# fudan-zvg/PARTNER

Measured on AMD Instinct MI355X. Metric: frames/sec polar voxelize+PFN+BEV+head, 30k-pt sweep (whole job), higher is better.
Workload: dtype f32

## Files before the change

### include/partner_hip.h

```cpp
#ifndef PARTNER_HIP_H
#define PARTNER_HIP_H

#include <stddef.h>
#include <stdint.h>

#ifdef __cplusplus
extern "C" {
#endif

#define PN_OK 0
#define PN_ERR_INVALID (-1)
#define PN_ERR_LAUNCH (-2)
#define PN_ERR_WORKSPACE (-3)

#define PN_ACT_NONE 0
#define PN_ACT_RELU 1
#define PN_ACT_TANH 2
#define PN_ACT_GELU 3

typedef void *pn_stream_t;

int pn_version(void);
int pn_last_error(char *buf, size_t buf_len);
int pn_device_count(void);
// ... 564 lines not shown
size_t pn_pillar_conv_packed_weight_floats(int cout, int cin);
int pn_pack_pillar_conv_weight_f32(const float *w_oihw, int cout, int cin, float *packed, pn_stream_t stream);
size_t pn_pillar_conv_workspace_bytes(int v_capacity, int batch, int oh, int ow, int cout);
int pn_pillar_conv3x3_f32(const float *canvas, int batch, int h, int w, int cin, int in_pixel_stride, int in_channel_offset,
                          const uint32_t *unq_keys, const int32_t *num_voxels, int v_capacity, int stride,
                          const float *packed_w, int cout, const float *scale, const float *shift, int act, float *out,
                          int out_pixel_stride, int out_channel_offset, void *workspace, size_t workspace_bytes,
                          pn_stream_t stream);
int pn_pillar_conv_planes_supported(int batch, int oh, int ow, int cout);
int pn_pillar_conv3x3_planes_f32(const float *canvas, int batch, int h, int w, int cin, int in_pixel_stride, int in_channel_offset,
                                 const uint32_t *unq_keys, const int32_t *num_voxels, int v_capacity, int stride,
                                 const float *packed_w, int cout, const float *scale, const float *shift, int act, float *planes,
                                 void *workspace, size_t workspace_bytes, pn_stream_t stream);
int pn_pillar_conv_rows_supported(int batch, int h, int w, int cin, int cout, int stride);
size_t pn_pillar_conv_rows_packed_weight_floats(int cout, int cin);
int pn_pack_pillar_conv_rows_weight_f32(const float *w_oihw, int cout, int cin, float *packed, pn_stream_t stream);
int pn_pillar_conv3x3_rows_f32(const float *canvas, int batch, int h, int w, int cin, int in_pixel_stride, int in_channel_offset,
                               const uint32_t *unq_keys, const int32_t *row_start, int v_capacity, const float *packed_rows_w, int cout,
                               const float *scale, const float *shift, int act, float *planes, float *out, int out_pixel_stride,
                               int out_channel_offset, pn_stream_t stream);
int pn_conv2d_nhwc_planes_supported(const pn_conv_desc *d);
int pn_conv2d_nhwc_planes_f32(const pn_conv_desc *d, const float *in, const float *packed_w, const float *scale, const float *shift,
                              float *planes, pn_stream_t stream);
size_t pn_pillar_pairs_bytes(int v_capacity, int batch, int oh, int ow);
int pn_pillar_pairs_build(const uint32_t *unq_keys, const int32_t *num_voxels, int v_capacity, int batch, int h, int w,
                          int stride, void *pair_tables, size_t table_bytes, pn_stream_t stream);
int pn_pillar_conv3x3_tables_f32(const float *canvas, int batch, int oh, int ow, int cin, int in_pixel_stride,
                                 int in_channel_offset, const void *pair_tables, int v_capacity, const float *packed_w,
                                 int cout, const float *scale, const float *shift, int act, float *out,
                                 int out_pixel_stride, int out_channel_offset, void *workspace, size_t workspace_bytes,
                                 pn_stream_t stream);
int pn_pillar_conv3x3_dgrad_f32(const float *dout, int batch, int oh, int ow, int cout, int dout_pixel_stride,
                                int dout_channel_offset, const void *pair_tables, const int32_t *num_voxels,
                                int v_capacity, const float *packed_wt, int cin, float *dfeat, void *workspace,
                                size_t workspace_bytes, pn_stream_t stream);
size_t pn_pillar_conv_wgrad_workspace_bytes(int v_capacity, int cin, int cout);
int pn_pillar_conv3x3_wgrad_f32(const float *canvas, int in_pixel_stride, int in_channel_offset, int cin, const float *dout,
                                int dout_pixel_stride, int dout_channel_offset, int cout, const void *pair_tables,
                                int v_capacity, int batch, int oh, int ow, float *dw_oihw, int accumulate, void *workspace,
                                size_t workspace_bytes, pn_stream_t stream);
size_t pn_conv_stat_partial_floats(const pn_conv_desc *desc, int tile);
int pn_conv2d_multi_f32(const pn_conv_job *jobs, int njobs, int tile, pn_stream_t stream);
int pn_conv2d_small_n_multi_f32(const pn_conv_job *jobs, int njobs, pn_stream_t stream);

int pn_conv3x3_tap_sum_f32(const float *g, int ldg, int batch, int h, int w, int cout, const float *scale,
                           const float *shift, int act, float *out, int out_pixel_stride,
// ... 53 lines not shown
```

### partner_amd/autodiff.py

```python
from __future__ import annotations

import os

import ctypes as C
from typing import Callable, List, Optional, Sequence

import torch

from . import hip, ops
from .routes import R


class Node:
    __slots__ = ("v", "g", "bw", "owned", "name", "needs_grad")

    def __init__(self, v: torch.Tensor, bw: Optional[Callable] = None, name: Optional[str] = None, needs_grad=True):
        self.v, self.bw, self.name, self.needs_grad = v, bw, name, needs_grad
        self.g: Optional[torch.Tensor] = None
        self.owned = False


class Tape:
    def __init__(self):
        self.nodes: List[Node] = []
# ... 304 lines not shown

    def bw(dy):
        dx = torch.empty_like(dy)
        hip.call("pn_l2_normalize_bwd_f32", y.data_ptr(), dy.data_ptr(), inv.data_ptr(), rows, c, float(eps), dx.data_ptr(), hip.stream())
        accumulate(x, dx, own=True)

    return t.new(y, bw)


def _pad4(dy: torch.Tensor) -> torch.Tensor:
    c = dy.shape[-1]
    if c % 4 == 0:
        return dy
    out = torch.zeros(dy.shape[:-1] + ((c + 3) // 4 * 4,), dtype=torch.float32, device=dy.device)
    out[..., :c].copy_(dy)
    return out




def conv2d(t: Tape, x: Node, w: Node, b: Optional[Node], stride=1, pad=0, relu=False) -> Node:
    wv = w.v
    cout, cin, k, _ = wv.shape
    layer = ops.ConvLayer(wv, stride=stride, pad=pad, shift=None if b is None else b.v, act=ops.ACT_RELU if relu else ops.ACT_NONE, wino4=R.train_wino4_max_pixels > 0)
    layer.wino4_max_pixels = R.train_wino4_max_pixels
    ct = x.v.shape[3]
    if ct != cin:
        layer.pad_input_channels(ct)
    y = layer(x.v)

    def bw(dy):
        if relu:
            dy = ops.relu_bwd(y, dy)
        dy4 = _pad4(dy)
        def weight_grads():
            dw = ops.conv_wgrad(x.v, dy4, k, k, stride, pad, cin=cin, cout=cout)
            accumulate(w, dw, own=True)
            if b is not None:
                accumulate(b, ops.channel_sum(dy4, c=cout), own=True)

        side_run(weight_grads, dy4, x.v)
        if x.needs_grad:
            dx = ops.ConvDgrad(wv, stride, pad)(dy4)
            if ct != cin:
                full = torch.zeros_like(x.v)
                full[..., :cin].copy_(dx)
                dx = full
# ... 131 lines not shown
```

### partner_amd/hip.py

```python
from __future__ import annotations

import ctypes as C
import os
from typing import Optional

import torch

_LIB_PATH = os.path.join(os.path.dirname(os.path.abspath(__file__)), "lib", "libpartner_hip.so")
_lib: Optional[C.CDLL] = None

ACT_NONE, ACT_RELU, ACT_TANH, ACT_GELU = 0, 1, 2, 3


class PartnerHipError(RuntimeError):
    pass


class ConvDesc(C.Structure):

    _fields_ = [(n, C.c_int32) for n in (
        "batch", "in_h", "in_w", "cin", "cout", "groups", "kh", "kw", "stride", "pad_h", "pad_w",
        "in_pixel_stride", "in_channel_offset", "out_pixel_stride", "out_channel_offset", "act", "deconv2x2",
        "range_strata", "pad_h_end", "pad_w_end", "accumulate", "frames_in_flight", "transpose_hw")]

# ... 156 lines not shown
                                      _F, _P, _F, _F, _F, _P, _P, _P, _P, _P, _P, _P, _P, _SZ, _P]),
    "pn_rotate_boxes_f32": (_I, [_P, _P, _I, _I, _I, C.c_double, _P]),
    "pn_split_polar_sectors_workspace_bytes": (_SZ, [_I, _I, _I]),
    "pn_split_polar_sectors_f32": (_I, [_P, _I, _I, _P, _I, _I, _P, _P, _P, _P, _P, _P, _P, _P, _SZ, _P]),
    "pn_assemble_rows_f32": (_I, [C.POINTER(RowPiece), _I, _I, _I, _I, _P, _I, _I, _P]),
    "pn_sparse_neighbors_transpose": (_I, [_P, _P, _I, _I, _I, _P, _P]),
    "pn_sparse_conv_wgrad_workspace_bytes": (_SZ, [_I, _I, _I, _I]),
    "pn_sparse_conv_wgrad_f32": (_I, [_P, _I, _I, _I, _P, _I, _P, _P, _I, _I, _P, _I, _P, _SZ, _P]),
    "pn_sparse_from_dense_nhwc": (_I, [_P, _P, _I, _P, _P, _I, _P, _P]),
    "pn_add_relu_f32": (_I, [_P, _P, _P, _SZ, _P]),
    "pn_pad_roll_f32": (_I, [_P, _I, _I, _I, _I, _I, _I, _I, _P, _P]),
    "pn_crop_roll_f32": (_I, [_P, _I, _I, _I, _I, _I, _I, _I, _P, _P]),
    "pn_scale_channels_f32": (_I, [_P, _P, _SZ, _I, _P, _P]),
    "pn_recip_clamp_f32": (_I, [_P, _F, _I, _P, _P]),
    "pn_recip_clamp_bwd_f32": (_I, [_P, _P, _F, _I, _P, _P]),
    "pn_global_augment_f32": (_I, [_P, _I, _I, _P, _I, _I, _I, _I, _I, _F, _F, _F, _F, _P, _P]),
    "pn_handle_create": (_I, [_I, _P]),
    "pn_handle_destroy": (_I, [_P]),
    "pn_handle_info": (_I, [_P, _P, _P, _P, _P, _P, _SZ]),
    "pn_handle_pci_bus_id": (_I, [_P, _P, _SZ]),
    "pn_conv3x3_tap_sum_f32": (_I, [_P, _I, _I, _I, _I, _I, _P, _P, _I, _P, _I, _I, _P]),
    "pn_conv2d_nhwc_planes_supported": (_I, [_P]),
    "pn_conv2d_nhwc_planes_f32": (_I, [_P, _P, _P, _P, _P, _P, _P]),
    "pn_comm_unique_id_bytes": (_SZ, []),
    "pn_comm_unique_id": (_I, [_P]),
    "pn_comm_create": (_I, [_P, _I, _I, _P]),
    "pn_comm_destroy": (_I, [_P]),
    "pn_allreduce_f32": (_I, [_P, _P, _P, _SZ, _I, _P]),
    "pn_broadcast_f32": (_I, [_P, _P, _SZ, _I, _P]),
    "pn_linear_packed_weight_floats": (_SZ, [_I, _I]),
    "pn_pack_linear_weight_f32": (_I, [_P, _I, _I, _P, _P]),
    "pn_linear_set_tile": (_I, [_I]),
    "pn_linear_f32": (_I, [_P, _I, _I, _I, _P, _I, _P, _I, _P, _I, _P, _I, _P]),
    "pn_linear_ksplit_f32": (_I, [_P, _I, _I, _I, _P, _I, _P, _I, _P, _I, _P, _I, _P]),
    "pn_linear_ln_f32": (_I, [_P, _I, _I, _I, _P, _I, _P, _I, _P, _I, _P, _I, _P, _P, _F, _P, _P]),
    "pn_conv_wino_packed_weight_floats": (_SZ, [_I, _I]),
    "pn_pack_conv_weight_wino_f32": (_I, [_P, _I, _I, _P, _P]),
    "pn_pack_conv_dgrad_weight_wino_f32": (_I, [_P, _I, _I, _P, _P]),
    "pn_pack_conv_dgrad_weight_wino4_f32": (_I, [_P, _I, _I, _P, _P]),
    "pn_conv2d_wino_nhwc_f32": (_I, [_P, _P, _P, _P, _P, _P, _P]),
    "pn_conv_wino4_packed_weight_floats": (_SZ, [_I, _I]),
    "pn_pack_conv_weight_wino4_f32": (_I, [_P, _I, _I, _P, _P]),
    "pn_conv_wino4_tiles": (_I, [_P]),
    "pn_conv2d_wino4_nhwc_f32": (_I, [_P, _P, _P, _P, _P, _P, _P]),
    "pn_wino4_planes_floats": (_SZ, [_I, _I, _I, _I]),
    "pn_wino4_planes_from_nhwc_f32": (_I, [_P, _I, _I, _I, _I, _I, _I, _I, _P, _P]),
# ... 140 lines not shown
```

### partner_amd/ops_conv.py

```python
from __future__ import annotations

import ctypes as C
from dataclasses import dataclass
from typing import Optional, Sequence, Tuple

import torch

from . import hip
from .hip import ACT_NONE, ACT_RELU, ACT_TANH, ConvDesc
from .ops_common import *
from .ops_common import _f32, _workspace
from .routes import R, S
from .ops_index import VoxelIndex



class frames_in_flight:

    def __init__(self, n: int):
        self.n, self.prev = max(1, int(n)), 1

    def __enter__(self):
        self.prev, S.frames_in_flight = S.frames_in_flight, self.n
        return self
# ... 57 lines not shown


def disable_conv_profiling() -> None:
    S.profiler = None


def _tap_pack(buf: torch.Tensor, tap_n: int, cout: int, cin: int):
    def pack(w, st):
        w9 = torch.zeros((tap_n, cin), dtype=torch.float32, device=w.device)
        w9[:9 * cout] = w.reshape(cout, -1, 9)[:, :cin].permute(2, 0, 1).reshape(9 * cout, -1)
        hip.call("pn_pack_linear_weight_f32", w9.data_ptr(), tap_n, cin, buf.data_ptr(), st)
    return pack


def _transposed_pack(layout: str, buf: torch.Tensor, cout: int, cin: int, keep: dict):
    def pack(w, st):
        keep[layout] = wt = w.detach().float().transpose(2, 3).contiguous()
        hip.call(f"pn_pack_conv_weight_{layout}_f32", wt.data_ptr(), cout, cin, buf.data_ptr(), st)
    return pack




class ConvLayer:

    def __init__(self, weight: torch.Tensor, stride=1, pad=0, groups=1, scale=None, shift=None, act=ACT_NONE,
                 deconv2x2=False, range_strata=0, dtype="f32", wino4=True):
        hip.require_device(weight)
        lib = hip.load()
        w = weight.detach().contiguous().float()
        dev = w.device
        st = hip.stream()
        self.deconv2x2, self.range_strata, self.groups = bool(deconv2x2), int(range_strata), int(groups)
        self.stride, self.act = int(stride), int(act)
        self.pad = (pad, pad) if isinstance(pad, int) else tuple(pad)
        assert dtype in ("f32", "bf16")
        self.dtype = dtype
        self.packed_rows = self.wino44_packed = None
        self.wino4_max_pixels = None
        self._chain_t, self._chain_t_src = {}, {}
        self._packs = PackedLayouts(w)
        if dtype == "bf16":
            if deconv2x2:
                cin, cout = w.shape[0], w.shape[1]
                assert tuple(w.shape[2:]) == (2, 2)
                self.cin, self.cout, self.kh, self.kw = cin, cout, 1, 1
                wc = w.permute(2, 3, 1, 0).reshape(4 * cout, cin, 1, 1).contiguous()
                self.packed = torch.empty(lib.pn_conv_packed_weight_bf16_elems(4 * cout, cin, 1, 1, 1), dtype=torch.bfloat16, device=dev)
                hip.call("pn_pack_conv_weight_bf16", wc.data_ptr(), 4 * cout, cin, 1, 1, 1, self.packed.data_ptr(), st)
                self._pack_bf16_rows(lib, wc, 4 * cout, cin, 1, 1, st)
            else:
                pack_groups = self.range_strata if self.range_strata > 1 else self.groups
                cout_t, cin_g, kh, kw = w.shape
                self.cin, self.cout, self.kh, self.kw = cin_g, cout_t // pack_groups, kh, kw
                self.packed = None
                self._bf16_general = (w, cout_t, cin_g, kh, kw, pack_groups)
                if pack_groups == 1:
                    self._pack_bf16_rows(lib, w, cout_t, cin_g, kh, kw, st)
                if self.packed_rows is None:
                    self._ensure_bf16_general()
        elif deconv2x2:
# ... 12 lines not shown
        self.shift = None if shift is None else shift.detach().contiguous().float()
        self.out_channels = self.cout * (self.groups if not deconv2x2 else 1)
        self._pack_cin = self.cin
        self.wino_packed = None
        if (dtype == "f32" and not deconv2x2 and self.range_strata <= 1 and self.groups == 1 and (self.kh, self.kw) == (3, 3)
                and self.stride == 1 and self.pad == (1, 1) and self.cin % 4 == 0 and R.conv_wino):
            self.wino_packed = _f32(lib.pn_conv_wino_packed_weight_floats(self.cout, self.cin), dev)
            self._packs.add("wino", pack_call("pn_pack_conv_weight_wino_f32", self.wino_packed, self.cout, self.cin), now=True)
        self.wino4_packed = None
        if self.wino_packed is not None and R.conv_wino4 and wino4 and self.cout % 32 == 0 and self.act in (ACT_NONE, ACT_RELU):
            self.wino4_packed = _f32(lib.pn_conv_wino4_packed_weight_floats(self.cout, self.cin), dev)
            self._packs.add("wino4", pack_call("pn_pack_conv_weight_wino4_f32", self.wino4_packed, self.cout, self.cin), now=True)
        self.wino24_packed = None
        if self.wino4_packed is not None and R.conv_chain2d and self.cin % 32 == 0:
            self.wino24_packed = _f32(lib.pn_conv_wino24_packed_weight_floats(self.cout, self.cin), dev)
            self._packs.add("wino24", pack_call("pn_pack_conv_weight_wino24_f32", self.wino24_packed, self.cout, self.cin), now=True)

        self.tap_packed = None
        if (dtype == "f32" and not deconv2x2 and self.range_strata <= 1 and self.groups == 1 and (self.kh, self.kw) == (3, 3) and self.stride == 1
                and self.pad == (1, 1) and self.cout <= 3 and self.cin >= 128 and self.cin % 4 == 0 and R.conv_tapsum and R.linear):
            self.tap_n = (9 * self.cout + 3) // 4 * 4
            self.tap_packed = _f32(lib.pn_linear_packed_weight_floats(self.tap_n, self.cin), dev)
            self._packs.add("tap", _tap_pack(self.tap_packed, self.tap_n, self.cout, self.cin), now=True)
        if self.wino24_packed is None:
            self._packs.weight = None

    def _ensure_bf16_general(self) -> None:
        if self.packed is None:
            w, cout_t, cin_g, kh, kw, pack_groups = self._bf16_general
            self.packed = torch.empty(hip.load().pn_conv_packed_weight_bf16_elems(self.cout, cin_g, kh, kw, pack_groups), dtype=torch.bfloat16,
                                      device=w.device)
            hip.call("pn_pack_conv_weight_bf16", w.data_ptr(), cout_t, cin_g, kh, kw, pack_groups, self.packed.data_ptr(), hip.stream())

    def _pack_bf16_rows(self, lib, w: torch.Tensor, rows: int, cin: int, kh: int, kw: int, st) -> None:
        if cin % 64 == 0 and self.cout % 16 == 0 and self.act in (ACT_NONE, ACT_RELU):
            self.packed_rows = torch.empty(lib.pn_conv_bf16_rows_packed_elems(rows, cin, kh, kw), dtype=torch.bfloat16, device=w.device)
            hip.call("pn_pack_conv_weight_bf16_rows", w.data_ptr(), rows, cin, kh, kw, self.packed_rows.data_ptr(), st)

    def planes_desc(self, b: int, h: int, w: int, ct: int, in_channel_offset: int = 0):
        if self.dtype != "f32" or self.deconv2x2 or self.range_strata > 1 or self.groups != 1 or not R.conv_planes:
            return None
        d = ConvDesc(b, h, w, self.cin, self.cout, 1, self.kh, self.kw, self.stride, self.pad[0], self.pad[1], ct, in_channel_offset, self.cout, 0,
                     self.act, 0, 0, 0, 0, 0)
        return d if hip.load().pn_conv2d_nhwc_planes_supported(C.byref(d)) else None

    def to_planes(self, x: torch.Tensor, planes: torch.Tensor, in_channel_offset: int = 0) -> None:
        hip.require_device(x, planes)
        b, h, w, ct = x.shape
        d = self.planes_desc(b, h, w, ct, in_channel_offset)
        assert d is not None, "ConvLayer.to_planes: check planes_desc first"
        self._packs.ensure("direct")
        oh, ow = self.out_hw(h, w)
        assert planes.numel() >= hip.load().pn_wino4_planes_floats(b, oh, ow, self.cout)
        st = hip.stream()
        prof = S.profiler
        if prof is not None:
            ev = prof.begin(st)
        hip.call("pn_conv2d_nhwc_planes_f32", C.byref(d), x.data_ptr(), self.packed.data_ptr(), hip.ptr(self.scale), hip.ptr(self.shift),
                 planes.data_ptr(), st)
        if prof is not None:
            prof.end(ev, 2.0 * b * oh * ow * self.cout * self.cin * self.kh * self.kw, st, tag=f"{oh}x{ow} {self.cin}->{self.cout} k{self.kh} -> planes")

    def chain_weights(self, layout: str, transposed: bool) -> torch.Tensor:
        cout, cin = self.cout, self._pack_cin
        if transposed:
            if layout not in self._chain_t:
                assert self._packs.weight is not None, "chain_weights: only layers with wino24_packed keep the weight the transposed layouts are packed from"
                buf = self._chain_t[layout] = _f32(getattr(hip.load(), f"pn_conv_{layout}_packed_weight_floats")(cout, cin), self.packed.device)
                self._packs.add(layout + "_t", _transposed_pack(layout, buf, cout, cin, self._chain_t_src))
            self._packs.pack(layout + "_t")
            return self._chain_t[layout]
        if layout == "wino44" and self.wino44_packed is None:
            assert self._packs.weight is not None, "chain_weights: only layers with wino24_packed keep the weight F(4,3)xF(4,3) is packed from"
            self.wino44_packed = _f32(hip.load().pn_conv_wino44_packed_weight_floats(cout, cin), self.packed.device)
            self._packs.add("wino44", pack_call("pn_pack_conv_weight_wino44_f32", self.wino44_packed, cout, cin))
        self._packs.ensure(layout)
# ... 48 lines not shown
            st = hip.stream()
            prof = S.profiler
            if prof is not None:
                ev = prof.begin(st)
            igemm = self.packed_rows is not None and hip.load().pn_conv2d_igemm_bf16_supported(C.byref(d)) == 1
            if igemm:
                hip.call("pn_conv2d_igemm_bf16", C.byref(d), x.data_ptr(), self.packed_rows.data_ptr(), hip.ptr(self.scale), hip.ptr(self.shift),
                         out.data_ptr(), int(out.dtype == torch.float32), st)
            else:
                if self.packed is None:
                    self._ensure_bf16_general()
                hip.call("pn_conv2d_nhwc_bf16", C.byref(d), x.data_ptr(), self.packed.data_ptr(), hip.ptr(self.scale), hip.ptr(self.shift),
                         out.data_ptr(), int(out.dtype == torch.float32), st)
            if prof is not None:
                macs = b * h * w * 4 * self.cout * self.cin if self.deconv2x2 else b * oh * ow * self.groups * self.cout * self.cin * self.kh * self.kw
                prof.end(ev, 2.0 * macs, st, tag=f"{oh}x{ow} {self.cin * self.groups}->{self.out_channels} k{self.kh} bf16")
            return out
        assert out.shape[:3] == ((b, ow, oh) if out_transposed else (b, oh, ow)) and out.is_contiguous()
        d = ConvDesc(b, h, w, self.cin, self.cout, self.groups, self.kh, self.kw, self.stride, self.pad[0], self.pad[1],
                     ct, in_channel_offset, out.shape[3], out_channel_offset, self.act, int(self.deconv2x2),
                     self.range_strata, 0, 0, int(accumulate))
        d.frames_in_flight = S.frames_in_flight
        d.transpose_hw = int(bool(out_transposed))
        st = hip.stream()
        prof = S.profiler
        if prof is not None:
            ev = prof.begin(st)
        use_tap = self.tap_packed is not None and not accumulate and self.cin == self._pack_cin and in_channel_offset % 4 == 0 and ct % 4 == 0
        use_wino4 = not use_tap and self._use_wino4(b, h, w, accumulate)
        use_wino = not use_tap and not use_wino4 and self._use_wino(b, h, w, accumulate)
        assert use_wino4 or not out_transposed, "ConvLayer: a transposed output needs the F(4,3) kernel (check _use_wino4 first)"
        self._packs.ensure("tap" if use_tap else "wino4" if use_wino4 else "wino" if use_wino else "direct")
        if use_tap:
            m = b * h * w
            g = torch.empty((m, self.tap_n), dtype=torch.float32, device=x.device)
            hip.call("pn_linear_ksplit_f32", x.data_ptr() + 4 * in_channel_offset, m, self.cin, ct, self.tap_packed.data_ptr(), self.tap_n, None, ACT_NONE,
                     None, self.tap_n, g.data_ptr(), self.tap_n, st)
            hip.call("pn_conv3x3_tap_sum_f32", g.data_ptr(), self.tap_n, b, h, w, self.cout, hip.ptr(self.scale), hip.ptr(self.shift), self.act,
                     out.data_ptr(), out.shape[3], out_channel_offset, st)
            if prof is not None:
                prof.end(ev, 2.0 * m * self.cout * self.cin * 9, st, tag=f"{oh}x{ow} {self.cin}->{self.out_channels} k3 gemm+taps", issued=2.0 * m * self.cin * 32)
            return out
        if use_wino4:
            hip.call("pn_conv2d_wino4_nhwc_f32", C.byref(d), x.data_ptr(), self.wino4_packed.data_ptr(), hip.ptr(self.scale), hip.ptr(self.shift),
                     out.data_ptr(), st)
        elif use_wino:
# ... 436 lines not shown
```

### partner_amd/routes.py

```python
from __future__ import annotations

import os
from contextlib import contextmanager


class Routes:
    def __init__(self):
        self.conv_wino = os.environ.get("PN_CONV_WINO", "1") != "0"
        self.conv_wino_min_tiles = int(os.environ.get("PN_CONV_WINO_MIN_TILES", "256"))
        self.conv_wino4 = os.environ.get("PN_CONV_WINO4", "1") != "0"
        self.conv_wino4_min_tiles = int(os.environ.get("PN_CONV_WINO4_MIN_TILES", "256"))
        self.conv_wino4_dgrad = os.environ.get("PN_CONV_WINO4_DGRAD", "1") != "0"
        self.conv_tapsum = os.environ.get("PN_CONV_TAPSUM", "1") != "0"
        self.conv_chain = os.environ.get("PN_CONV_CHAIN", "1") != "0"
        self.conv_chain2d = os.environ.get("PN_CONV_CHAIN2D", "1") != "0"
        self.conv_chain44 = os.environ.get("PN_CONV_CHAIN44", "1") != "0"
        self.conv_planes = os.environ.get("PN_CONV_PLANES", "1") != "0"
        self.conv_wgrad_wino4 = os.environ.get("PN_CONV_WGRAD_WINO4", "1") != "0"
        self.conv_wgrad_wino4_min_quads = int(os.environ.get("PN_CONV_WGRAD_WINO4_MIN_QUADS", "4096"))
        self.pillar_conv = os.environ.get("PN_PILLAR_CONV", "1") != "0"
        self.pillar_planes = os.environ.get("PN_PILLAR_PLANES", "1") != "0"
        self.pillar_rows = os.environ.get("PN_PILLAR_ROWS", "1") != "0"
        self.pillar_conv_max_fill = float(os.environ.get("PN_PILLAR_CONV_MAX_FILL", "0.35"))
        self.pillar_rows_max_fill = float(os.environ.get("PN_PILLAR_ROWS_MAX_FILL", "1.25"))
        self.fused_sweeps = os.environ.get("PN_FUSED_SWEEPS", "1") != "0"
        self.sample_streams = os.environ.get("PN_SAMPLE_STREAMS", "1") != "0"
        self.pfn_clears_index = os.environ.get("PN_PFN_CLEARS_INDEX", "1") != "0"
        self.linear = os.environ.get("PN_LINEAR", "1") != "0"
        self.ln_fold = os.environ.get("PN_LN_FOLD", "1") != "0"
        self.head_chain = os.environ.get("PN_HEAD_CHAIN", "1") != "0"
        self.sparse_c16 = os.environ.get("PN_SPARSE_C16", "1") != "0"
        self.sparse_row_bits = os.environ.get("PN_SPARSE_ROW_BITS", "1") != "0"
        self.sparse_grouped = os.environ.get("PN_SPARSE_GROUPED", "1") != "0"
        self.sparse_struct_stream = os.environ.get("PN_SPARSE_STRUCT_STREAM", "1") != "0"
        self.train_wgrad_stream = os.environ.get("PN_TRAIN_WGRAD_STREAM", "1") != "0"
        self.train_wino4_max_pixels = int(os.environ.get("PN_TRAIN_WINO4_MAX_PIXELS", "16384"))
        self.train_pillar_conv = os.environ.get("PN_TRAIN_PILLAR_CONV", "1") != "0"
        self.train_prepack = os.environ.get("PN_TRAIN_PREPACK", "1") != "0"
        self.train_chain_max_pixels = int(os.environ.get("PN_TRAIN_CHAIN_MAX_PIXELS", "4096"))
        self.train_strat_expand = os.environ.get("PN_TRAIN_STRAT_EXPAND", "0") != "0"

# ... 24 lines not shown
```

### partner_amd/train.py

```python
from __future__ import annotations

import math
import os
from typing import Dict, List, Optional, Sequence, Tuple

import numpy as np
import torch
from torch import nn

from . import hip, ops
from .routes import R
from .heads import CenterHeadSingle, CenterHeadSinglePos, RangeStratified
from .nn_utils import RSNorm
from .readers import DynamicPFNet

RELU, NONE, TANH = ops.ACT_RELU, ops.ACT_NONE, ops.ACT_TANH


def one_cycle(step: int, total_step: int, lr_max: float, moms: Sequence[float], div_factor: float, pct_start: float):
    a1 = int(total_step * pct_start)
    low = lr_max / div_factor

    def cos(start, end, pct):
        return end + (start - end) / 2 * (math.cos(math.pi * pct) + 1)
# ... 74 lines not shown
    for n, o, k in zip(names, offs, nums):
        dst, shape = ps.offsets[n]
        if shape.numel() != k:
            raise ValueError(f"optimizer state: parameter {n} has {k} elements in the checkpoint, {shape.numel()} in the model")
        ps.flat_m[dst:dst + k].copy_(m_src[o:o + k])
        ps.flat_v[dst:dst + k].copy_(v_src[o:o + k])
    return int(state["iter"])




class _Conv:

    def __init__(self, ps: ParamStore, wname: str, bname: Optional[str], stride=1, pad=0, act=NONE, transposed=False,
                 cin_pad: Optional[int] = None):
        self.ps, self.wname, self.bname = ps, wname, bname
        w = ps.p[wname]
        self.stride, self.pad, self.act, self.transposed = stride, pad, act, transposed
        self.k = w.shape[2]
        if transposed:
            self.layer = ops.ConvLayer(w, deconv2x2=True, act=act)
            self.dgrad = ops.ConvLayer(w, stride=2, pad=0)
        else:
            self.layer = ops.ConvLayer(w, stride=stride, pad=pad, shift=None if bname is None else ps.p[bname], act=act, wino4=R.train_wino4_max_pixels > 0)
            self.layer.wino4_max_pixels = R.train_wino4_max_pixels
            if cin_pad is not None:
                self.layer.pad_input_channels(cin_pad)
            self.dgrad = ops.ConvDgrad(w, stride, pad)
        self.cin_real = w.shape[1] if not transposed else w.shape[0]
        self.x = None
        self.in_co = 0
        ps.convs.append(self)

    def prepack_fwd(self, token):
        self.layer.repack(self.ps.p[self.wname], None if self.bname is None else self.ps.p[self.bname], token=token)
        self.layer.prepack_used()

    def prepack_bwd(self, token):
        self.dgrad.repack(self.ps.p[self.wname], token=token)
        self.dgrad.prepack_used()

    def _chain_ok(self, t, layer) -> bool:
        return (R.train_chain_max_pixels > 0 and not self.transposed and self.k == 3 and self.stride == 1 and self.pad == 1
                and t.shape[1] * t.shape[2] <= R.train_chain_max_pixels and t.shape[3] == layer.cin
                and ops.conv_chain_supported([layer], t.shape[0], t.shape[1], t.shape[2]))

    def fwd(self, x, out=None, out_co=0, in_co=0):
# ... 607 lines not shown
```

Before: 1836.

## Add polynomial-transform MFMA kernel for stride-2 3x3 convolutions

Adds a new HIP kernel for 3x3 stride-2 pad-1 convolutions. It applies a Winograd-like polynomial transform to the input along the width, so each output quad needs fewer multiplies. The kernel runs on MFMA 32x32x2 f32, double-buffers A and B, and can write straight to wino4 planes for the next layer. Routing is gated by a tile-count threshold and support checks, and training paths opt out. The risk is worse f32 accuracy from the transform, plus added complexity and a possible shape-dependent slowdown on small layers.

Result: no change. 1837, median of 4 (+0.0%).

```diff
diff --git a/include/partner_hip.h b/include/partner_hip.h
--- a/include/partner_hip.h
+++ b/include/partner_hip.h
@@ -610,6 +610,11 @@
 int pn_conv2d_nhwc_planes_supported(const pn_conv_desc *d);
 int pn_conv2d_nhwc_planes_f32(const pn_conv_desc *d, const float *in, const float *packed_w, const float *scale, const float *shift,
                               float *planes, pn_stream_t stream);
+size_t pn_conv_s2poly_packed_weight_floats(int cout, int cin);
+int pn_pack_conv_weight_s2poly_f32(const float *w_oihw, int cout, int cin, float *packed, pn_stream_t stream);
+int pn_conv2d_s2poly_supported(const pn_conv_desc *d);
+int pn_conv2d_s2poly_f32(const pn_conv_desc *d, const float *in, const float *packed_w, const float *scale, const float *shift,
+                         float *out, float *planes, pn_stream_t stream);
 size_t pn_pillar_pairs_bytes(int v_capacity, int batch, int oh, int ow);
 int pn_pillar_pairs_build(const uint32_t *unq_keys, const int32_t *num_voxels, int v_capacity, int batch, int h, int w,
                           int stride, void *pair_tables, size_t table_bytes, pn_stream_t stream);
diff --git a/partner_amd/autodiff.py b/partner_amd/autodiff.py
--- a/partner_amd/autodiff.py
+++ b/partner_amd/autodiff.py
@@ -350,7 +350,7 @@
 def conv2d(t: Tape, x: Node, w: Node, b: Optional[Node], stride=1, pad=0, relu=False) -> Node:
     wv = w.v
     cout, cin, k, _ = wv.shape
-    layer = ops.ConvLayer(wv, stride=stride, pad=pad, shift=None if b is None else b.v, act=ops.ACT_RELU if relu else ops.ACT_NONE, wino4=R.train_wino4_max_pixels > 0)
+    layer = ops.ConvLayer(wv, stride=stride, pad=pad, shift=None if b is None else b.v, act=ops.ACT_RELU if relu else ops.ACT_NONE, wino4=R.train_wino4_max_pixels > 0, s2poly=False)
     layer.wino4_max_pixels = R.train_wino4_max_pixels
     ct = x.v.shape[3]
     if ct != cin:
diff --git a/partner_amd/csrc/conv_s2poly.hip b/partner_amd/csrc/conv_s2poly.hip
--- /dev/null
+++ b/partner_amd/csrc/conv_s2poly.hip
@@ -0,0 +1,385 @@
+#include "pn_common.h"
+#include "wino_planes.h"
+#include <algorithm>
+#include <cstdlib>
+#include <type_traits>
+
+namespace {
+
+using f32x16 = __attribute__((ext_vector_type(16))) float;
+using f32x4 = __attribute__((ext_vector_type(4))) float;
+
+constexpr int SP_N = 32;
+constexpr int SP_NPAD = 64;
+constexpr int SP_Q = 32;
+constexpr int SP_LD = 36;
+constexpr int SP_POS = 9;
+constexpr int SP_WSETS = 6;
+constexpr int SP_STAGE = SP_POS * SP_Q * SP_LD;
+constexpr int sp_join(int cw) { return cw * (4 / cw) * (4 / cw - 1) * 4 * (16 / (4 / cw) / 4) * 64 * 4; }
+constexpr int sp_tld(int cw) { return SP_N * cw + 4; }
+constexpr size_t sp_smem() { return (size_t)2 * SP_STAGE * sizeof(float); }
+static_assert(sp_join(1) + 4 * SP_Q * sp_tld(1) <= 2 * SP_STAGE && sp_join(2) + 4 * SP_Q * sp_tld(2) <= 2 * SP_STAGE,
+              "the join buffer and the finished tile reuse the stages");
+
+struct S2PolyArgs {
+  const float* in;
+  const float* w;
+  const float* scale;
+  const float* shift;
+  float* out;
+  float* planes;
+  int H, W, OH, OW, Cin, Cout;
+  int in_ps, in_co, out_ps, out_co;
+  int act;
+  int Wq, tiles, ncol;
+  int chunks, cout_pad;
+  unsigned in_bytes, w_bytes, plane_floats;
+};
+
+template <int CW>
+__global__ __launch_bounds__(256, 1) void conv_s2poly_kernel(S2PolyArgs a) {
+  constexpr int KS = 4 / CW;
+  constexpr int CPW = 32 / KS;
+  constexpr int NF = CPW / 8;
+  constexpr int R = 16 / KS, R4 = R / 4;
+  constexpr int BN = SP_N * CW;
+  constexpr int SP_JOIN = sp_join(CW), SP_TLD = sp_tld(CW);
+  extern __shared__ __attribute__((aligned(16))) float smem[];
+  const int tid = threadIdx.x, lane = tid & 63, wv = __builtin_amdgcn_readfirstlane(tid >> 6);
+  const int cw = wv % CW, kq = wv / CW;
+  const int li = lane & 31, lh = lane >> 5;
+  const int per_xcd = gridDim.x >> 3;
+  const int tl = (blockIdx.x & 7) * per_xcd + (blockIdx.x >> 3);
+  if (tl >= a.tiles) return;
+  const int pt = tl / a.ncol, n0 = (tl - pt * a.ncol) * BN;
+  const int pl = tid >> 3, c4 = tid & 7;
+
+  const long long back = ((long long)a.W + 1) * a.in_ps;
+  unsigned a_off, a_off0, a_rmask = 0;
+  {
+    const int p = pt * SP_Q + pl;
+    const int rowi = p / a.Wq, oq = p - rowi * a.Wq;
+    const int b = rowi / a.OH, oh = rowi - b * a.OH;
+    const long long pix = ((long long)b * a.H + (2 * oh - 1)) * a.W + (8 * oq - 1);
+    a_off = (unsigned)((pix * a.in_ps + back + a.in_co + c4 * 4) * 4);
+    a_off0 = oq > 0 ? a_off : 0xffffffffu;
+    for (int kh = 0; kh < 3; ++kh)
+      if ((unsigned)(2 * oh + kh - 1) < (unsigned)a.H) a_rmask |= 1u << kh;
+  }
+  const unsigned b_base = (unsigned)((((size_t)(CPW / 4) * kq + lh) * a.cout_pad + n0 + cw * SP_N + li) * 16);
+  const int col = n0 + cw * SP_N + li;
+  const float sc = (a.scale && col < a.Cout) ? a.scale[col] : 1.f;
+  const float sh = (a.shift && col < a.Cout) ? a.shift[col] : 0.f;
+  const __amdgpu_buffer_rsrc_t rsrc_a = __builtin_amdgcn_make_buffer_rsrc(reinterpret_cast<char*>(const_cast<float*>(a.in)) - back * 4, 0,
+                                                                         a.in_bytes + (unsigned)(back * 4), 0x00020000);
+  const __amdgpu_buffer_rsrc_t rsrc_b = __builtin_amdgcn_make_buffer_rsrc(const_cast<float*>(a.w), 0, a.w_bytes, 0x00020000);
+  const int nsteps = 3 * a.chunks;
+  const unsigned cp16 = (unsigned)a.cout_pad * 16u;
+  const unsigned ps4 = (unsigned)a.in_ps * 4u;
+  int ld_kh = 0, ld_chunk = 0, lb_kh = 0, lb_chunk = 0;
+
+  f32x4 ra[2][9];
+  auto load_a = [&](bool live, f32x4 (&ra)[9]) {
+    const unsigned so_a = (unsigned)((ld_kh * a.W * a.in_ps + ld_chunk * 32) * 4);
+    const bool rok = live & (ld_chunk * 32 + c4 * 4 < a.Cin) & (((a_rmask >> ld_kh) & 1u) != 0);
+#pragma unroll
+    for (int j = 0; j < 9; ++j)
+      ra[j] = __builtin_bit_cast(f32x4, __builtin_amdgcn_raw_buffer_load_b128(rsrc_a, rok ? (j == 0 ? a_off0 : a_off) : 0xffffffffu, so_a + (unsigned)j * ps4, 0));
+    if (++ld_kh == 3) { ld_kh = 0; ++ld_chunk; }
+  };
+  auto store_a = [&](int stage, const f32x4 (&ra)[9]) {
+    float* As = smem + stage * SP_STAGE + pl * SP_LD + c4 * 4;
+    const f32x4 c2 = {2.f, 2.f, 2.f, 2.f}, m2 = {-2.f, -2.f, -2.f, -2.f}, m3 = {-3.f, -3.f, -3.f, -3.f};
+    const f32x4 d0 = ra[0], d1 = ra[2], d2 = ra[4], d3 = ra[6], d4 = ra[8];
+    const f32x4 s = d3 - d1, t = d0 - d2;
+    f32x4 v[SP_POS];
+    v[0] = __builtin_elementwise_fma(c2, t, s);
+    v[1] = __builtin_elementwise_fma(m2, d1, d3 - d2);
+    v[2] = __builtin_elementwise_fma(c2, d1, __builtin_elementwise_fma(m3, d2, d3));
+    v[3] = s;
+    v[4] = __builtin_elementwise_fma(m2, s, d4 - d2);
+    v[5] = ra[1]; v[6] = ra[3]; v[7] = ra[5]; v[8] = ra[7];
+#pragma unroll
+    for (int q = 0; q < SP_POS; ++q) *reinterpret_cast<f32x4*>(As + q * SP_Q * SP_LD) = v[q];
+  };
+  f32x16 acc[SP_POS];
+  const int a_frag = li * SP_LD + lh * 4 + kq * CPW;
+  f32x4 af[SP_POS][NF], bf[2][SP_WSETS][NF];
+  auto read_a = [&](int stage) {
+#pragma unroll
+    for (int q = 0; q < SP_POS; ++q)
+#pragma unroll
+      for (int f = 0; f < NF; ++f) af[q][f] = *reinterpret_cast<const f32x4*>(smem + stage * SP_STAGE + a_frag + f * 8 + q * SP_Q * SP_LD);
+  };
+  auto load_b = [&](bool live, f32x4 (&f)[SP_WSETS][NF]) {
+    const unsigned so_b = (unsigned)((lb_chunk * 3 + lb_kh) * (SP_WSETS * 8)) * cp16;
+    const unsigned vo = live ? b_base : 0xffffffffu;
+#pragma unroll
+    for (int q = 0; q < SP_WSETS; ++q)
+#pragma unroll
+      for (int g = 0; g < NF; ++g)
+        f[q][g] = __builtin_bit_cast(f32x4, __builtin_amdgcn_raw_buffer_load_b128(rsrc_b, vo, so_b + (unsigned)(q * 8 + 2 * g) * cp16, 0));
+    if (++lb_kh == 3) { lb_kh = 0; ++lb_chunk; }
+  };
+  auto kstep = [&](auto par_c, int t) __attribute__((always_inline)) {
+    constexpr int buf = decltype(par_c)::value;
+    __syncthreads();
+    read_a(buf);
+    load_b(t + 1 < nsteps, bf[buf ^ 1]);
+#pragma unroll
+    for (int f = 0; f < NF; ++f)
+#pragma unroll
+      for (int kk = 0; kk < 4; ++kk) {
+#pragma unroll
+        for (int q = 0; q < 5; ++q) acc[q] = __builtin_amdgcn_mfma_f32_32x32x2f32(af[q][f][kk], bf[buf][q][f][kk], acc[q], 0, 0, 0);
+#pragma unroll
+        for (int q = 5; q < SP_POS; ++q) acc[q] = __builtin_amdgcn_mfma_f32_32x32x2f32(af[q][f][kk], bf[buf][5][f][kk], acc[q], 0, 0, 0);
+      }
+    load_a(t + 2 < nsteps, ra[buf]);
+    store_a(buf ^ 1, ra[buf ^ 1]);
+#pragma unroll
+    for (int k = 0; k < SP_POS * NF; ++k) __builtin_amdgcn_sched_group_barrier(0x100, 1, 0);
+#pragma unroll
+    for (int k = 0; k < SP_WSETS * NF; ++k) {
+      __builtin_amdgcn_sched_group_barrier(0x008, 2, 0);
+      __builtin_amdgcn_sched_group_barrier(0x020, 1, 0);
+    }
+#pragma unroll
+    for (int k = 0; k < SP_POS; ++k) {
+      __builtin_amdgcn_sched_group_barrier(0x008, NF, 0);
+      __builtin_amdgcn_sched_group_barrier(0x002, 4, 0);
+      __builtin_amdgcn_sched_group_barrier(0x020, 1, 0);
+    }
+#pragma unroll
+    for (int k = 0; k < SP_POS; ++k) {
+      __builtin_amdgcn_sched_group_barrier(0x008, NF, 0);
+      __builtin_amdgcn_sched_group_barrier(0x002, 8, 0);
+      __builtin_amdgcn_sched_group_barrier(0x200, 1, 0);
+    }
+    __builtin_amdgcn_sched_barrier(0);
+  };
+  using I0 = std::integral_constant<int, 0>;
+  using I1 = std::integral_constant<int, 1>;
+  using I2 = std::integral_constant<int, 2>;
+  using I3 = std::integral_constant<int, 3>;
+  using JCW = std::integral_constant<int, CW>;
+
+  auto finish = [&](auto d_c) __attribute__((always_inline)) {
+    constexpr int D = decltype(d_c)::value;
+#pragma unroll
+    for (int r = 0; r < 16; ++r) {
+      const float m0 = acc[0][r], m1 = acc[1][r], m2 = acc[2][r], m3 = acc[3][r], m4 = acc[4][r];
+      const float s12 = m1 + m2, d12 = m1 - m2;
+      acc[5][r] += (m0 + s12) + m3;
+      acc[6][r] += d12 + 2.f * m3;
+      acc[7][r] += s12 + 4.f * m3;
+      acc[8][r] += (d12 + 8.f * m3) + m4;
+    }
+    f32x4* J = reinterpret_cast<f32x4*>(smem) + (size_t)cw * (KS * (KS - 1) * 4 * R4 * 64) + lane;
+#pragma unroll
+    for (int d = 0; d < KS; ++d) {
+      if (d == D) continue;
+      const int sl = D < d ? D : D - 1;
+#pragma unroll
+      for (int y = 0; y < 4; ++y)
+#pragma unroll
+        for (int g = 0; g < R4; ++g) {
+          const int r0 = R * d + 4 * g;
+          const f32x4 v = {acc[5 + y][r0], acc[5 + y][r0 + 1], acc[5 + y][r0 + 2], acc[5 + y][r0 + 3]};
+          J[(((d * (KS - 1) + sl) * 4 + y) * R4 + g) * 64] = v;
+        }
+    }
+    __syncthreads();
+    float* T = smem + SP_JOIN;
+    const float lo = a.act == PN_ACT_RELU ? 0.f : -__builtin_inff();
+#pragma unroll
+    for (int y = 0; y < 4; ++y)
+#pragma unroll
+      for (int g = 0; g < R4; ++g) {
+        const int r0 = R * D + 4 * g;
+        f32x4 s = {acc[5 + y][r0], acc[5 + y][r0 + 1], acc[5 + y][r0 + 2], acc[5 + y][r0 + 3]};
+#pragma unroll
+        for (int sl = 0; sl < KS - 1; ++sl) s += J[(((D * (KS - 1) + sl) * 4 + y) * R4 + g) * 64];
+#pragma unroll
+        for (int rr = 0; rr < 4; ++rr) {
+          const int ql = rr + 8 * (r0 >> 2) + 4 * lh;
+          T[(4 * ql + y) * SP_TLD + cw * SP_N + li] = fmaxf(fmaf(s[rr], sc, sh), lo);
+        }
+      }
+  };
+
+  load_a(true, ra[0]);
+  load_b(true, bf[0]);
+#pragma unroll
+  for (int q = 0; q < SP_POS; ++q)
+#pragma unroll
+    for (int r = 0; r < 16; ++r) acc[q][r] = 0.f;
+  load_a(nsteps > 1, ra[1]);
+  store_a(0, ra[0]);
+  for (int t = 0; t < nsteps; t += 2) {
+    kstep(I0{}, t);
+    if (t + 1 < nsteps) kstep(I1{}, t + 1);
+  }
+  __syncthreads();
+  if constexpr (JCW::value == 1) {
+    if (kq == 0) finish(I0{});
+    else if (kq == 1) finish(I1{});
+    else if (kq == 2) finish(I2{});
+    else finish(I3{});
+  } else {
+    if (kq == 0) finish(I0{});
+    else finish(I1{});
+  }
+  __syncthreads();
+
+#pragma unroll
+  for (int it = 0; it < CW; ++it) {
+    const int item = tid + 256 * it;
+    const int q = a.planes ? (item & 31) : item / (8 * CW), c4l = a.planes ? (item >> 5) : item % (8 * CW);
+    const int gn = n0 + 4 * c4l;
+    if (gn >= a.Cout) continue;
+    const int p = pt * SP_Q + q;
+    const int rowi = p / a.Wq, xq = p - rowi * a.Wq;
+    const float* T = smem + SP_JOIN + 4 * c4l;
+    f32x4 d[6];
+#pragma unroll
+    for (int i = 0; i < 6; ++i) {
+      const bool inside = (i > 0 || xq > 0) && (i < 5 || xq + 1 < a.Wq);
+      const f32x4 v = *reinterpret_cast<const f32x4*>(T + (inside ? 4 * q - 1 + i : 4 * q) * SP_TLD);
+      const f32x4 z = {0.f, 0.f, 0.f, 0.f};
+      d[i] = inside ? v : z;
+    }
+    if (a.out) {
+      float* o = a.out + ((size_t)rowi * a.OW + 4 * xq) * a.out_ps + a.out_co + gn;
+#pragma unroll
+      for (int i = 0; i < 4; ++i) *reinterpret_cast<f32x4*>(o + (size_t)i * a.out_ps) = d[1 + i];
+    }
+    if (a.planes) {
+      const int img = rowi / a.OH, r = rowi - img * a.OH;
+      f32x4 vv[6];
+      pn::wino4_input_transform4(d, vv);
+      pn::wino4_store_planes(a.planes, vv, gn >> 2, a.Cout >> 2, a.plane_floats, img, r, xq, a.OH, a.Wq);
+    }
+  }
+}
+
+__global__ void pack_s2poly_weight_kernel(const float* __restrict__ w, int cout, int cin, int cout_pad, float* __restrict__ packed, size_t total) {
+  for (size_t i = blockIdx.x * (size_t)blockDim.x + threadIdx.x; i < total; i += (size_t)gridDim.x * blockDim.x) {
+    size_t r = i;
+    const int k1 = r & 3; r >>= 2;
+    const int n = (int)(r % cout_pad); r /= cout_pad;
+    const int k4 = r & 7; r >>= 3;
+    const int q = (int)(r % SP_WSETS); r /= SP_WSETS;
+    const int kh = (int)(r % 3);
+    const int chunk = (int)(r / 3);
+    const int c = chunk * 32 + k4 * 4 + k1;
+    double v = 0.0;
+    if (n < cout && c < cin) {
+      const float* g = w + (((size_t)n * cin + c) * 3 + kh) * 3;
+      const double g0 = g[0], g1 = g[1], g2 = g[2];
+      v = q == 0 ? g0 / 2.0 : q == 1 ? -(g0 + g2) / 2.0 : q == 2 ? (g2 - g0) / 6.0 : q == 3 ? g0 / 6.0 + g2 / 3.0 : q == 4 ? g2 : g1;
+    }
+    packed[i] = (float)v;
+  }
+}
+
+int s2poly_form(int qtiles, int cout, int ncu) {
+  const char* e = getenv("PN_S2POLY_COLS");
+  if (e && (e[0] == '1' || e[0] == '2') && !e[1]) return e[0] - '0';
+  const long long r1 = pn::cdiv((long long)qtiles * pn::cdiv(cout, SP_N), ncu), r2 = pn::cdiv((long long)qtiles * pn::cdiv(cout, 2 * SP_N), ncu);
+  return r2 * 17 < r1 * 10 ? 2 : 1;
+}
+
+}
+
+extern "C" {
+
+size_t pn_conv_s2poly_packed_weight_floats(int cout, int cin) {
+  if (cout < 1 || cin < 1) return 0;
+  return (size_t)pn::cdiv(cin, 32) * 3 * SP_WSETS * 8 * (size_t)(pn::cdiv(cout, SP_NPAD) * SP_NPAD) * 4;
+}
+
+int pn_pack_conv_weight_s2poly_f32(const float* w_oihw, int cout, int cin, float* packed, pn_stream_t stream) {
+  PN_REQUIRE(w_oihw && packed && cout >= 1 && cin >= 1, "pack_conv_weight_s2poly: bad arguments");
+  const size_t total = pn_conv_s2poly_packed_weight_floats(cout, cin);
+  hipLaunchKernelGGL(pack_s2poly_weight_kernel, dim3((unsigned)std::min<size_t>(4096, (total + 255) / 256)), dim3(256), 0, pn::S(stream), w_oihw, cout, cin,
+                     pn::cdiv(cout, SP_NPAD) * SP_NPAD, packed, total);
+  return pn::check_launch("pack_s2poly_weight_kernel");
+}
+
+int pn_conv2d_s2poly_supported(const pn_conv_desc* d) {
+  if (!d) return 0;
+  if (!(d->kh == 3 && d->kw == 3 && d->stride == 2 && d->pad_h == 1 && d->pad_w == 1 && d->groups == 1 && !d->deconv2x2 && d->range_strata <= 1 &&
+        !d->accumulate && d->pad_h_end == 0 && d->pad_w_end == 0 && !d->transpose_hw))
+    return 0;
+  if (d->batch < 1 || d->in_h < 1 || d->in_w < 8 || d->in_w % 8) return 0;
+  const int wq = d->in_w / 8, oh = (d->in_h - 1) / 2 + 1;
+  if (wq > SP_Q || (wq & (wq - 1))) return 0;
+  if (((long long)d->batch * oh * wq) % SP_Q) return 0;
+  if (d->cin < 4 || d->cin % 4 || d->cout < 4 || d->cout % 4) return 0;
+  if (d->in_pixel_stride % 4 || d->in_channel_offset % 4 || d->out_pixel_stride % 4 || d->out_channel_offset % 4 || d->in_channel_offset < 0 ||
+      d->out_channel_offset < 0)
+    return 0;
+  if (d->in_pixel_stride < d->in_channel_offset + d->cin || d->out_pixel_stride < d->out_channel_offset + d->cout) return 0;
+  if (!(d->act == PN_ACT_NONE || d->act == PN_ACT_RELU)) return 0;
+  const unsigned long long in_bytes = (unsigned long long)d->batch * d->in_h * d->in_w * d->in_pixel_stride * 4ull;
+  if (in_bytes + ((unsigned long long)d->in_w + 1) * d->in_pixel_stride * 4ull >= (1ull << 32)) return 0;
+  if ((long long)d->batch * oh * wq / SP_Q * pn::cdiv(d->cout, SP_N) >= (1ll << 30)) return 0;
+  return 1;
+}
+
+int pn_conv2d_s2poly_f32(const pn_conv_desc* d, const float* in, const float* packed_w, const float* scale, const float* shift, float* out, float* planes,
+                         pn_stream_t stream) {
+  PN_REQUIRE(d && in && packed_w && (out || planes), "conv_s2poly: null pointer");
+  PN_REQUIRE(pn_conv2d_s2poly_supported(d),
+             "conv_s2poly: not covered (3x3 / stride 2 / pad 1, one group, input width % 8 == 0, output rows of 4 .. 128 pixels filling whole 32-quad "
+             "tiles, cin / cout / strides / offsets % 4 == 0, activation none or ReLU)");
+  PN_REQUIRE(((uintptr_t)in & 15) == 0 && ((uintptr_t)packed_w & 15) == 0 && ((uintptr_t)out & 15) == 0 && ((uintptr_t)planes & 15) == 0,
+             "conv_s2poly: pointers must be 16-byte aligned");
+  S2PolyArgs a{};
+  a.in = in; a.w = packed_w; a.scale = scale; a.shift = shift; a.out = out; a.planes = planes;
+  a.H = d->in_h; a.W = d->in_w; a.OH = (d->in_h - 1) / 2 + 1; a.OW = d->in_w / 2; a.Cin = d->cin; a.Cout = d->cout;
+  a.in_ps = d->in_pixel_stride; a.in_co = d->in_channel_offset; a.out_ps = d->out_pixel_stride; a.out_co = d->out_channel_offset;
+  a.act = d->act;
+  a.Wq = a.OW / 4;
+  a.chunks = pn::cdiv(d->cin, 32);
+  a.cout_pad = pn::cdiv(d->cout, SP_NPAD) * SP_NPAD;
+  const int qtiles = (int)((long long)d->batch * a.OH * a.Wq / SP_Q);
+  static int cus[64] = {0};
+  int dev = 0;
+  (void)hipGetDevice(&dev);
+  if (dev >= 0 && dev < 64 && cus[dev] == 0) {
+    int n = 0;
+    cus[dev] = (hipDeviceGetAttribute(&n, hipDeviceAttributeMultiprocessorCount, dev) == hipSuccess && n >= 8) ? n : 256;
+  }
+  const int cw = s2poly_form(qtiles, d->cout, (dev >= 0 && dev < 64) ? cus[dev] : 256);
+  a.ncol = pn::cdiv(d->cout, SP_N * cw);
+  a.tiles = qtiles * a.ncol;
+  a.in_bytes = (unsigned)((unsigned long long)d->batch * d->in_h * d->in_w * d->in_pixel_stride * 4ull);
+  a.w_bytes = (unsigned)(pn_conv_s2poly_packed_weight_floats(d->cout, d->cin) * 4);
+  if (planes) {
+    const size_t pf = pn_wino4_planes_floats(d->batch, a.OH, a.OW, d->cout);
+    PN_REQUIRE(pf > 0 && pf * 4ull < (1ull << 32), "conv_s2poly: planes need cout % 8 == 0 and a map of less than 4 GB");
+    a.plane_floats = (unsigned)((size_t)d->batch * (a.OH + 2) * a.Wq * 4);
+  }
+  static bool attr_done[64] = {false};
+  if (pn::first_use_on_device(attr_done)) {
+    (void)hipFuncSetAttribute(reinterpret_cast<const void*>(&conv_s2poly_kernel<1>), hipFuncAttributeMaxDynamicSharedMemorySize, (int)sp_smem());
+    (void)hipFuncSetAttribute(reinterpret_cast<const void*>(&conv_s2poly_kernel<2>), hipFuncAttributeMaxDynamicSharedMemorySize, (int)sp_smem());
+  }
+  const dim3 grid((unsigned)(pn::cdiv(a.tiles, 8) * 8));
+  hipStream_t st = pn::S(stream);
+  pn::ProfileSlot ps;
+  const bool prof = pn::take_profile_slot(ps);
+  if (cw == 2) {
+    if (prof) hipExtLaunchKernelGGL(conv_s2poly_kernel<2>, grid, dim3(256), sp_smem(), st, ps.start, ps.stop, 0, a);
+    else hipLaunchKernelGGL(conv_s2poly_kernel<2>, grid, dim3(256), sp_smem(), st, a);
+  } else {
+    if (prof) hipExtLaunchKernelGGL(conv_s2poly_kernel<1>, grid, dim3(256), sp_smem(), st, ps.start, ps.stop, 0, a);
+    else hipLaunchKernelGGL(conv_s2poly_kernel<1>, grid, dim3(256), sp_smem(), st, a);
+  }
+  return pn::check_launch("conv_s2poly_kernel");
+}
+
+}
diff --git a/partner_amd/hip.py b/partner_amd/hip.py
--- a/partner_amd/hip.py
+++ b/partner_amd/hip.py
@@ -202,6 +202,10 @@
     "pn_conv3x3_tap_sum_f32": (_I, [_P, _I, _I, _I, _I, _I, _P, _P, _I, _P, _I, _I, _P]),
     "pn_conv2d_nhwc_planes_supported": (_I, [_P]),
     "pn_conv2d_nhwc_planes_f32": (_I, [_P, _P, _P, _P, _P, _P, _P]),
+    "pn_conv_s2poly_packed_weight_floats": (_SZ, [_I, _I]),
+    "pn_pack_conv_weight_s2poly_f32": (_I, [_P, _I, _I, _P, _P]),
+    "pn_conv2d_s2poly_supported": (_I, [_P]),
+    "pn_conv2d_s2poly_f32": (_I, [_P, _P, _P, _P, _P, _P, _P, _P]),
     "pn_comm_unique_id_bytes": (_SZ, []),
     "pn_comm_unique_id": (_I, [_P]),
     "pn_comm_create": (_I, [_P, _I, _I, _P]),
diff --git a/partner_amd/ops_conv.py b/partner_amd/ops_conv.py
--- a/partner_amd/ops_conv.py
+++ b/partner_amd/ops_conv.py
@@ -103,10 +103,14 @@
 
 
 
+def _s2poly_faster(b: int, oh: int, ow: int, cin: int, cout: int) -> bool:
+    return (b * oh * (ow // 4) // 32) * ((cout + 31) // 32) >= R.conv_s2poly_min_tiles
+
+
 class ConvLayer:
 
     def __init__(self, weight: torch.Tensor, stride=1, pad=0, groups=1, scale=None, shift=None, act=ACT_NONE,
-                 deconv2x2=False, range_strata=0, dtype="f32", wino4=True):
+                 deconv2x2=False, range_strata=0, dtype="f32", wino4=True, s2poly=True):
         hip.require_device(weight)
         lib = hip.load()
         w = weight.detach().contiguous().float()
@@ -117,7 +121,8 @@
         self.pad = (pad, pad) if isinstance(pad, int) else tuple(pad)
         assert dtype in ("f32", "bf16")
         self.dtype = dtype
-        self.packed_rows = self.wino44_packed = None
+        self.packed_rows = self.wino44_packed = self.s2poly_packed = None
+        self.s2poly_ok = False
         self.wino4_max_pixels = None
         self._chain_t, self._chain_t_src = {}, {}
         self._packs = PackedLayouts(w)
@@ -176,7 +181,9 @@
             self.tap_n = (9 * self.cout + 3) // 4 * 4
             self.tap_packed = _f32(lib.pn_linear_packed_weight_floats(self.tap_n, self.cin), dev)
             self._packs.add("tap", _tap_pack(self.tap_packed, self.tap_n, self.cout, self.cin), now=True)
-        if self.wino24_packed is None:
+        self.s2poly_ok = (s2poly and dtype == "f32" and not deconv2x2 and self.range_strata <= 1 and self.groups == 1 and (self.kh, self.kw) == (3, 3)
+                          and self.stride == 2 and self.pad == (1, 1) and self.cin % 4 == 0 and self.cout % 4 == 0 and self.act in (ACT_NONE, ACT_RELU))
+        if self.wino24_packed is None and not self.s2poly_ok:
             self._packs.weight = None
 
     def _ensure_bf16_general(self) -> None:
@@ -191,9 +198,47 @@
             self.packed_rows = torch.empty(lib.pn_conv_bf16_rows_packed_elems(rows, cin, kh, kw), dtype=torch.bfloat16, device=w.device)
             hip.call("pn_pack_conv_weight_bf16_rows", w.data_ptr(), rows, cin, kh, kw, self.packed_rows.data_ptr(), st)
 
+    def _s2poly_desc(self, b: int, h: int, w: int, ct: int, in_channel_offset: int, out_ps: int, out_co: int):
+        if not (self.s2poly_ok and R.conv_s2poly and self.cin == self._pack_cin):
+            return None
+        d = ConvDesc(b, h, w, self.cin, self.cout, 1, 3, 3, 2, 1, 1, ct, in_channel_offset, out_ps, out_co, self.act, 0, 0, 0, 0, 0)
+        if not hip.load().pn_conv2d_s2poly_supported(C.byref(d)) or not _s2poly_faster(b, (h - 1) // 2 + 1, w // 2, self.cin, self.cout):
+            return None
+        return d
+
+    def _s2poly_weights(self) -> torch.Tensor:
+        if self.s2poly_packed is None:
+            self.s2poly_packed = _f32(hip.load().pn_conv_s2poly_packed_weight_floats(self.cout, self._pack_cin), self.packed.device)
+            self._packs.add("s2poly", pack_call("pn_pack_conv_weight_s2poly_f32", self.s2poly_packed, self.cout, self._pack_cin))
+        self._packs.ensure("s2poly")
+        return self.s2poly_packed
+
+    def _s2poly(self, d, x: torch.Tensor, out: Optional[torch.Tensor], planes: Optional[torch.Tensor]) -> None:
+        wp = self._s2poly_weights()
+        oh, ow = self.out_hw(d.in_h, d.in_w)
+        st = hip.stream()
+        prof = S.profiler
+        if prof is not None:
+            ev = prof.begin(st)
+        hip.call("pn_conv2d_s2poly_f32", C.byref(d), x.data_ptr(), wp.data_ptr(), hip.ptr(self.scale), hip.ptr(self.shift), hip.ptr(out), hip.ptr(planes), st)
+        if prof is not None:
+            flops = 2.0 * d.batch * oh * ow * self.cout * self.cin * 9
+            prof.end(ev, flops, st, tag=f"{oh}x{ow} {self.cin}->{self.cout} k3 s2poly{'' if planes is None else ' -> planes'}", issued=0.75 * flops)
+
     def planes_desc(self, b: int, h: int, w: int, ct: int, in_channel_offset: int = 0):
+        return self._planes_route(b, h, w, ct, in_channel_offset)[0]
+
+    def _planes_route(self, b: int, h: int, w: int, ct: int, in_channel_offset: int):
         if self.dtype != "f32" or self.deconv2x2 or self.range_strata > 1 or self.groups != 1 or not R.conv_planes:
-            return None
+            return None, False
+        if self.cout % 8 == 0:
+            d = self._s2poly_desc(b, h, w, ct, in_channel_offset, self.cout, 0)
+            if d is not None:
+                return d, True
+        d = self._direct_planes_desc(b, h, w, ct, in_channel_offset)
+        return d, False
+
+    def _direct_planes_desc(self, b: int, h: int, w: int, ct: int, in_channel_offset: int):
         d = ConvDesc(b, h, w, self.cin, self.cout, 1, self.kh, self.kw, self.stride, self.pad[0], self.pad[1], ct, in_channel_offset, self.cout, 0,
                      self.act, 0, 0, 0, 0, 0)
         return d if hip.load().pn_conv2d_nhwc_planes_supported(C.byref(d)) else None
@@ -201,11 +246,14 @@
     def to_planes(self, x: torch.Tensor, planes: torch.Tensor, in_channel_offset: int = 0) -> None:
         hip.require_device(x, planes)
         b, h, w, ct = x.shape
-        d = self.planes_desc(b, h, w, ct, in_channel_offset)
+        d, poly = self._planes_route(b, h, w, ct, in_channel_offset)
         assert d is not None, "ConvLayer.to_planes: check planes_desc first"
-        self._packs.ensure("direct")
         oh, ow = self.out_hw(h, w)
         assert planes.numel() >= hip.load().pn_wino4_planes_floats(b, oh, ow, self.cout)
+        if poly:
+            self._s2poly(d, x, None, planes)
+            return
+        self._packs.ensure("direct")
         st = hip.stream()
         prof = S.profiler
         if prof is not None:
@@ -300,6 +348,11 @@
                      self.range_strata, 0, 0, int(accumulate))
         d.frames_in_flight = S.frames_in_flight
         d.transpose_hw = int(bool(out_transposed))
+        if self.s2poly_ok and not accumulate and not out_transposed:
+            dp = self._s2poly_desc(b, h, w, ct, in_channel_offset, out.shape[3], out_channel_offset)
+            if dp is not None:
+                self._s2poly(dp, x, out, None)
+                return out
         st = hip.stream()
         prof = S.profiler
         if prof is not None:
diff --git a/partner_amd/routes.py b/partner_amd/routes.py
--- a/partner_amd/routes.py
+++ b/partner_amd/routes.py
@@ -16,7 +16,9 @@
         self.conv_chain2d = os.environ.get("PN_CONV_CHAIN2D", "1") != "0"
         self.conv_chain44 = os.environ.get("PN_CONV_CHAIN44", "1") != "0"
         self.conv_planes = os.environ.get("PN_CONV_PLANES", "1") != "0"
-        self.conv_wgrad_wino4 = os.environ.get("PN_CONV_WGRAD_WINO4", "1") != "0"
+        self.conv_s2poly = os.environ.get("PN_CONV_S2POLY", "1") != "0"
+        self.conv_s2poly_min_tiles = int(os.environ.get("PN_CONV_S2POLY_MIN_TILES", "256"))
+        self.conv_wgrad_wino4 =os.environ.get("PN_CONV_WGRAD_WINO4", "1") != "0"
         self.conv_wgrad_wino4_min_quads = int(os.environ.get("PN_CONV_WGRAD_WINO4_MIN_QUADS", "4096"))
         self.pillar_conv = os.environ.get("PN_PILLAR_CONV", "1") != "0"
         self.pillar_planes = os.environ.get("PN_PILLAR_PLANES", "1") != "0"
diff --git a/partner_amd/train.py b/partner_amd/train.py
--- a/partner_amd/train.py
+++ b/partner_amd/train.py
@@ -120,7 +120,7 @@
             self.layer = ops.ConvLayer(w, deconv2x2=True, act=act)
             self.dgrad = ops.ConvLayer(w, stride=2, pad=0)
         else:
-            self.layer = ops.ConvLayer(w, stride=stride, pad=pad, shift=None if bname is None else ps.p[bname], act=act, wino4=R.train_wino4_max_pixels > 0)
+            self.layer = ops.ConvLayer(w, stride=stride, pad=pad, shift=None if bname is None else ps.p[bname], act=act, wino4=R.train_wino4_max_pixels > 0, s2poly=False)
             self.layer.wino4_max_pixels = R.train_wino4_max_pixels
             if cin_pad is not None:
                 self.layer.pad_input_channels(cin_pad)
```
